# FFmpeg/FFmpeg

Hardware: AMD Instinct MI355X
Metric: swscale_nv12_1080p_to_4k_bicubic_Mpixels_per_s (higher is better)
Workload: dtype u8

## Files before the change

ffmpeg_amd/csrc/kernels/sws_up2.hip:

```cpp
#include <stdlib.h>
#include <type_traits>
#include <vector>

#include "common.h"
#include "sws_kernels.h"

typedef uint32_t up_u2 __attribute__((ext_vector_type(2)));
typedef uint32_t up_u3 __attribute__((ext_vector_type(3)));
typedef uint32_t up_u4 __attribute__((ext_vector_type(4)));
typedef uint32_t up_u8 __attribute__((ext_vector_type(8)));
typedef up_u3 __attribute__((aligned(4))) up_u3a;
typedef const uint8_t __attribute__((address_space(1))) *up_gcp;
typedef uint8_t __attribute__((address_space(1))) *up_gp;
typedef const up_u3a __attribute__((address_space(1))) *up_gc3;
typedef up_u2 __attribute__((address_space(1))) *up_g2;
typedef up_u4 __attribute__((aligned(4))) up_u4a;
typedef up_u2 __attribute__((aligned(4))) up_u2a;
typedef const up_u4a __attribute__((address_space(1))) *up_gc4;
typedef const up_u2a __attribute__((address_space(1))) *up_gc2;
typedef up_u4a __attribute__((address_space(1))) *up_g4;
typedef const up_u8 __attribute__((address_space(4))) *up_cc8;

struct UpRaw { uint32_t q[3]; };
struct UpRawH { uint32_t q[6]; };
// ... 217 lines not shown
#pragma unroll
    for (int i = 0; i < 8; i++)
        hprev[i] = 0;
    int kround = HB ? 1 << (vsh - 1) : 64 << 12;
    asm volatile("" : "+v"(kround));

    auto hpass = [&](const Raw &w, uint32_t (&Pnew)[8]) {
        int h[8];
        if (HB) {
            uint32_t v[6];
            constexpr int NQ = PAIR ? 6 : 4;
#pragma unroll
            for (int i = 0; i < NQ; i++)
                v[i] = w.q[i];
            if (border) {
                if (PAIR) {
                    const uint32_t q0 = w.q[0], q1 = w.q[1], q2 = w.q[2], q3 = w.q[3], q4 = w.q[4], q5 = w.q[5];
                    v[0] = lb ? q0 : rb ? q2 : q0; v[1] = lb ? q0 : rb ? q3 : q1; v[2] = lb ? q0 : rb ? q4 : q2;
                    v[3] = lb ? q1 : rb ? q5 : q3; v[4] = lb ? q2 : rb ? q5 : q4; v[5] = lb ? q3 : rb ? q5 : q5;
                } else {
                    const uint32_t q0 = w.q[0], q1 = w.q[1], q2 = w.q[2], q3 = w.q[3];
                    const uint32_t f0 = __builtin_amdgcn_perm(q0, q0, 0x01000100u), f3 = __builtin_amdgcn_perm(q3, q3, 0x03020302u);
                    v[0] = lb ? f0 : rb ? q1 : q0; v[1] = lb ? q0 : rb ? q2 : q1;
                    v[2] = lb ? q1 : rb ? q3 : q2; v[3] = lb ? q2 : rb ? f3 : q3;
                }
            }
            if (smsb) {
                typedef unsigned short up_h2 __attribute__((ext_vector_type(2)));
#pragma unroll
                for (int i = 0; i < NQ; i++)
                    v[i] = __builtin_bit_cast(uint32_t, __builtin_bit_cast(up_h2, v[i]) >> (unsigned short)smsb);
            }
            if (PAIR) {
                uint32_t a[5], b[5];
#pragma unroll
                for (int k = 0; k < 5; k++) {
                    a[k] = __builtin_amdgcn_perm(v[k + 1], v[k], 0x05040100u);
                    b[k] = __builtin_amdgcn_perm(v[k + 1], v[k], 0x07060302u);
                }
                int ha[4], hb[4];
                up_h4s(ha, a[0], a[1], a[1], a[2], a[2], a[3], a[3], a[4], cf, hsh);
                up_h4s(hb, b[0], b[1], b[1], b[2], b[2], b[3], b[3], b[4], cf, hsh);
#pragma unroll
                for (int i = 0; i < 4; i++) {
                    h[2 * i] = ha[i];
                    h[2 * i + 1] = hb[i];
                }
            } else {
                const uint32_t p0 = v[0], p2 = v[1], p4 = v[2], p6 = v[3];
                const uint32_t p1 = __builtin_amdgcn_alignbyte(v[1], v[0], 2), p3 = __builtin_amdgcn_alignbyte(v[2], v[1], 2);
                const uint32_t p5 = __builtin_amdgcn_alignbyte(v[3], v[2], 2);
                int hl[4], hh[4];
                up_h4s(hl, p0, p1, p1, p2, p2, p3, p3, p4, cf, hsh);
                up_h4s(hh, p2, p3, p3, p4, p4, p5, p5, p6, cf + 8, hsh);
#pragma unroll
                for (int i = 0; i < 4; i++) {
                    h[i] = hl[i];
                    h[4 + i] = hh[i];
                }
            }
#pragma unroll
            for (int i = 0; i < 8; i++) {
                Pnew[i] = __builtin_bit_cast(uint32_t, __builtin_amdgcn_cvt_pk_i16(hprev[i], h[i]));
                hprev[i] = h[i];
            }
            return;
        }
        uint32_t v0 = w.q[0], v1 = w.q[1], v2 = w.q[2];
        if (border) {
            const uint32_t f0 = __builtin_amdgcn_perm(w.q[0], w.q[0], fixl), f2 = __builtin_amdgcn_perm(w.q[2], w.q[2], fixr);
            v0 = lb ? f0 : rb ? w.q[1] : w.q[0];
            v1 = lb ? w.q[0] : rb ? w.q[2] : w.q[1];
            v2 = lb ? w.q[1] : rb ? f2 : w.q[2];
        }
        if (PAIR) {
            const uint32_t a0 = __builtin_amdgcn_perm(v1, v0, sA0), a1 = __builtin_amdgcn_perm(v1, v0, sA1);
            const uint32_t a2 = __builtin_amdgcn_perm(v1, v0, sA2), a3 = __builtin_amdgcn_perm(v2, v1, sA1);
            const uint32_t a4 = __builtin_amdgcn_perm(v2, v1, sA2);
            const uint32_t b0 = __builtin_amdgcn_perm(v1, v0, sB0), b1 = __builtin_amdgcn_perm(v1, v0, sB1);
            const uint32_t b2 = __builtin_amdgcn_perm(v1, v0, sB2), b3 = __builtin_amdgcn_perm(v2, v1, sB1);
            const uint32_t b4 = __builtin_amdgcn_perm(v2, v1, sB2);
            int ha[4], hb[4];
            if (SC) {
                up_h4c(ha, a0, a1, a1, a2, a2, a3, a3, a4, cE0, cE1, cO0, cO1);
                up_h4c(hb, b0, b1, b1, b2, b2, b3, b3, b4, cE0, cE1, cO0, cO1);
                if (border) {
                    const uint32_t *L = J.hco + 4, *R = J.hco + 10;
                    const int l0 = up_h1(a0, a2, L[0], L[1]), l1 = up_h1(a1, a3, L[2], L[3]), l2 = up_h1(a1, a3, L[4], L[5]);
                    const int m0 = up_h1(b0, b2, L[0], L[1]), m1 = up_h1(b1, b3, L[2], L[3]), m2 = up_h1(b1, b3, L[4], L[5]);
                    const int r1 = up_h1(a1, a3, R[0], R[1]), r2 = up_h1(a1, a3, R[2], R[3]), r3 = up_h1(a2, a4, R[4], R[5]);
                    const int q1 = up_h1(b1, b3, R[0], R[1]), q2 = up_h1(b1, b3, R[2], R[3]), q3 = up_h1(b2, b4, R[4], R[5]);
                    ha[0] = lb ? l0 : ha[0]; ha[1] = lb ? l1 : rb ? r1 : ha[1]; ha[2] = lb ? l2 : rb ? r2 : ha[2]; ha[3] = rb ? r3 : ha[3];
                    hb[0] = lb ? m0 : hb[0]; hb[1] = lb ? m1 : rb ? q1 : hb[1]; hb[2] = lb ? m2 : rb ? q2 : hb[2]; hb[3] = rb ? q3 : hb[3];
                }
            } else {
                up_h4(ha, a0, a1, a1, a2, a2, a3, a3, a4, cf);
                up_h4(hb, b0, b1, b1, b2, b2, b3, b3, b4, cf);
            }
#pragma unroll
            for (int i = 0; i < 4; i++) {
                h[2 * i] = ha[i];
                h[2 * i + 1] = hb[i];
            }
        } else {
            const uint32_t p0 = __builtin_amdgcn_perm(v1, v0, 0x0c030c02u), p1 = __builtin_amdgcn_perm(v1, v0, 0x0c040c03u);
            const uint32_t p2 = __builtin_amdgcn_perm(v1, v0, 0x0c050c04u), p3 = __builtin_amdgcn_perm(v1, v0, 0x0c060c05u);
            const uint32_t p4 = __builtin_amdgcn_perm(v1, v0, 0x0c070c06u), p5 = __builtin_amdgcn_perm(v2, v1, 0x0c040c03u);
            const uint32_t p6 = __builtin_amdgcn_perm(v2, v1, 0x0c050c04u);
            int hl[4], hh[4];
            if (SC) {
                up_h4c(hl, p0, p1, p1, p2, p2, p3, p3, p4, cE0, cE1, cO0, cO1);
                up_h4c(hh, p2, p3, p3, p4, p4, p5, p5, p6, cE0, cE1, cO0, cO1);
                if (border) {
                    const uint32_t *L = J.hco + 4, *R = J.hco + 10;
                    const int l0 = up_h1(p0, p2, L[0], L[1]), l1 = up_h1(p1, p3, L[2], L[3]), l2 = up_h1(p1, p3, L[4], L[5]);
                    const int r5 = up_h1(p3, p5, R[0], R[1]), r6 = up_h1(p3, p5, R[2], R[3]), r7 = up_h1(p4, p6, R[4], R[5]);
                    hl[0] = lb ? l0 : hl[0]; hl[1] = lb ? l1 : hl[1]; hl[2] = lb ? l2 : hl[2];
                    hh[1] = rb ? r5 : hh[1]; hh[2] = rb ? r6 : hh[2]; hh[3] = rb ? r7 : hh[3];
                }
            } else {
                up_h4(hl, p0, p1, p1, p2, p2, p3, p3, p4, cf);
                up_h4(hh, p2, p3, p3, p4, p4, p5, p5, p6, cf + 8);
            }
#pragma unroll
            for (int i = 0; i < 4; i++) {
                h[i] = hl[i];
                h[4 + i] = hh[i];
            }
        }
        if (RC) {
            const int rcc = J.rc_coeff, rco = J.rc_offset;
#pragma unroll
            for (int i = 0; i < 8; i++)
                h[i] = (__mul24(min(h[i], 32767), rcc) + rco) >> 14;
        }
#pragma unroll
        for (int i = 0; i < 8; i++) {
            Pnew[i] = __builtin_bit_cast(uint32_t, __builtin_amdgcn_cvt_pk_i16(hprev[i], h[i]));
            hprev[i] = h[i];
        }
    };

    Raw buf[D];
#pragma unroll
    for (int k = 0; k < D; k++)
        load_next(buf[k]);
#pragma unroll
    for (int k = 0; k < 3; k++) {
        hpass(buf[k % D], ring[k]);
        load_next(buf[k % D]);
    }

    const uint32_t *vt = J.vfv;
    for (int r = a; r < b; r += 6) {
        up_u8 c8[3];
#pragma unroll
        for (int q = 0; q < 3; q++)
            c8[q] = *(up_cc8)(vt + 4 * (r + 2 * q) - 4);
#pragma unroll
        for (int k = 0; k < 6; k++) {
            Raw &w = buf[(k + 3) % D];
            if constexpr (HB != 0) {
                const bool live = act && r + k < b;
                hpass(w, ring[k % 3]);
                const up_u8 cc = c8[k >> 1];
                const uint32_t fb01 = k & 1 ? cc.s4 : cc.s0, fb23 = k & 1 ? cc.s5 : cc.s1;
                const uint32_t fa01 = k & 1 ? cc.s6 : cc.s2, fa23 = k & 1 ? cc.s7 : cc.s3;
                const int y = 2 * (r + k) - 3;
                typedef unsigned short up_h2 __attribute__((ext_vector_type(2)));
                uint32_t o0[4], o1[4];
                up_v8h(o0, ring[(k + 1) % 3], ring[k % 3], fb01, fb23, kround, vsh, maxpk);
                uint32_t off = doff;
                asm volatile("" : "+v"(off));
#pragma unroll
                for (int i = 0; i < 4; i++)
                    o0[i] = __builtin_bit_cast(uint32_t, __builtin_bit_cast(up_h2, o0[i]) << (unsigned short)dmsb);
                if (live && y >= 0) {
                    up_u4 st; st.x = o0[0]; st.y = o0[1]; st.z = o0[2]; st.w = o0[3];
                    if (NTS) __builtin_nontemporal_store(st, (up_g4)((up_gp)dr + off));
                    else *(up_g4)((up_gp)dr + off) = st;
                }
                up_v8h(o1, ring[(k + 1) % 3], ring[k % 3], fa01, fa23, kround, vsh, maxpk);
#pragma unroll
                for (int i = 0; i < 4; i++)
                    o1[i] = __builtin_bit_cast(uint32_t, __builtin_bit_cast(up_h2, o1[i]) << (unsigned short)dmsb);
                if (live && y + 1 < dstH) {
                    up_u4 st; st.x = o1[0]; st.y = o1[1]; st.z = o1[2]; st.w = o1[3];
                    if (NTS) __builtin_nontemporal_store(st, (up_g4)((up_gp)(dr + dstride) + off));
                    else *(up_g4)((up_gp)(dr + dstride) + off) = st;
                }
                dr += 2 * dstride;
                asm("" : "+s"(dr));
                load_next(w);
                continue;
            }
            if (r + k < b) {
                if (!DBG_COPY)
                    hpass(w, ring[k % 3]);
                const up_u8 cc = c8[k >> 1];
                const uint32_t fb01 = k & 1 ? cc.s4 : cc.s0, fb23 = k & 1 ? cc.s5 : cc.s1;
                const uint32_t fa01 = k & 1 ? cc.s6 : cc.s2, fa23 = k & 1 ? cc.s7 : cc.s3;
                const int y = 2 * (r + k) - 3;
                uint32_t w0, w1, a0, a1;
                if (DBG_COPY) { w0 = w.q[0] + fb01; w1 = w.q[1] + fb23; a0 = w.q[1] + fa01; a1 = w.q[2] + fa23; }
                else up_v8(w0, w1, ring[(k + 1) % 3], ring[k % 3], fb01, fb23, kround);
                uint32_t off = doff;
                asm volatile("" : "+v"(off));
                if (act && y >= 0 && (!DBG_NOST || (w0 == 0x12345678u && w1 == 0x9abcdef0u))) {
                    up_u2 s; s.x = w0; s.y = w1;
                    if (NTS) __builtin_nontemporal_store(s, (up_g2)((up_gp)dr + off));
                    else *(up_g2)((up_gp)dr + off) = s;
                }
                if (!DBG_COPY)
                    up_v8(a0, a1, ring[(k + 1) % 3], ring[k % 3], fa01, fa23, kround);
                if (act && y + 1 < dstH && (!DBG_NOST || (a0 == 0x12345678u && a1 == 0x9abcdef0u))) {
                    up_u2 s; s.x = a0; s.y = a1;
                    if (NTS) __builtin_nontemporal_store(s, (up_g2)((up_gp)(dr + dstride) + off));
                    else *(up_g2)((up_gp)(dr + dstride) + off) = s;
                }
                dr += 2 * dstride;
                asm("" : "+s"(dr));
            }
            load_next(w);
        }
    }
}

template <int D, int VAR, int HB = 0, int RC = 0, int SC = 0>
__global__ __launch_bounds__(256) void k_sws_up2(FFHipUp2Args A)
{
    const int wave = __builtin_amdgcn_readfirstlane((int)(threadIdx.x >> 6));
    const int lane = threadIdx.x & 63;
    const uint32_t blk = sws_block_numbering(blockIdx.x, gridDim.x, A.xcd);
    const uint32_t gw = blk * 4u + (uint32_t)wave;
    if (gw >= (uint32_t)A.units_per_pack * (uint32_t)A.npacks)
        return;
    const int pack = (int)(gw / (uint32_t)A.units_per_pack);
    const int u = (int)(gw - (uint32_t)pack * (uint32_t)A.units_per_pack);
    int j = 0;
    if (A.njobs > 1 && u >= A.job[1].unit_begin) j = 1;
    if (A.njobs > 2 && u >= A.job[2].unit_begin) j = 2;
    const FFHipUp2Job &J = A.job[j];
    const int local = u - J.unit_begin;
    const int strip = local / J.upj, idx = local - strip * J.upj;
    const int nf = J.nfull << A.fshift;
    int frame0 = pack << A.fshift, fsh = 0, gbase;
    if (idx < nf) {
        const int fsub = idx / J.nfull;
        frame0 += fsub;
        gbase = (idx - fsub * J.nfull) * 64;
        if (frame0 >= A.nframes)
            return;
    } else {
        fsh = A.fshift;
        gbase = J.nfull * 64 + (idx - nf) * (64 >> fsh);
    }
    if (J.pair)
        up2_unit<1, D, VAR, HB, RC, SC>(J, frame0, fsh, gbase, strip, lane, A.nframes);
    else
        up2_unit<0, D, VAR, HB, RC, SC>(J, frame0, fsh, gbase, strip, lane, A.nframes);
}


int ffhip_up2_virtual_bank(const int16_t *filter, const int32_t *pos, int n_dst, int n_src, std::vector<uint32_t> *out)
{
    if (n_dst != 2 * n_src || n_src < 4)
        return 0;
    out->assign((size_t)n_dst * 2, 0);
    for (int x = 0; x < n_dst; x++) {
        const int s0 = (x >> 1) - 2 + (x & 1);
        int16_t v[4] = { 0, 0, 0, 0 };
        bool used[4] = { false, false, false, false };
        for (int i = 0; i < 4; i++) {
            const int16_t c = filter[(size_t)x * 4 + i];
            if (!c)
                continue;
            const int p = pos[x] + i;
            if (p < 0 || p >= n_src)
                return 0;
            int k = 0;
            for (; k < 4; k++) {
                int q = s0 + k;
                q = q < 0 ? 0 : q >= n_src ? n_src - 1 : q;
                if (q == p && !used[k])
                    break;
            }
            if (k == 4)
                return 0;
            used[k] = true;
            v[k] = c;
        }
        (*out)[2 * (size_t)x] = (uint16_t)v[0] | ((uint32_t)(uint16_t)v[1] << 16);
        (*out)[2 * (size_t)x + 1] = (uint16_t)v[2] | ((uint32_t)(uint16_t)v[3] << 16);
    }
    return 1;
}

int ffhip_up2_hco(const std::vector<uint32_t> &v, uint32_t out[16])
{
    const int n = (int)(v.size() / 2);
    if (n < 16 || (n & 1))
        return 0;
    for (int x = 3; x < n - 3; x++)
        if (v[2 * (size_t)x] != v[2 * (size_t)(4 + (x & 1))] || v[2 * (size_t)x + 1] != v[2 * (size_t)(4 + (x & 1)) + 1])
            return 0;
    for (int i = 0; i < 4; i++)
        out[i] = v[8 + i];
    for (int i = 0; i < 6; i++) {
        out[4 + i] = v[i];
        out[10 + i] = v[2 * (size_t)(n - 3) + i];
    }
    return 1;
}

void ffhip_up2_plan_job(FFHipUp2Job *j, int lanes_per_frame, int want)
{
    const int steps = j->srcH + 1;
    int n = cdiv(steps, want);
    int s = cdiv(cdiv(steps, n), 6) * 6;
    j->steps_per_strip = s;
    j->nstrips = cdiv(steps, s);
    if (lanes_per_frame == 64) {
        j->nfull = 0;
        j->upj = cdiv(j->ngroups, 64);
    } else {
        j->nfull = j->ngroups / 64;
        j->upj = j->nfull * (64 / lanes_per_frame) + cdiv(j->ngroups - j->nfull * 64, lanes_per_frame);
    }
}

int ffhip_launch_up2(FFHipUp2Args &A, int depth, int var, hipStream_t stream)
{
    if (A.nframes <= 0)
        return 0;
    int u = 0;
    for (int i = 0; i < A.njobs; i++) {
        A.job[i].unit_begin = u;
        u += A.job[i].upj * A.job[i].nstrips;
    }
    A.units_per_pack = u;
    A.npacks = (A.nframes + (1 << A.fshift) - 1) >> A.fshift;
    const long long waves = (long long)u * A.npacks;
    if (waves >= (1LL << 31)) {
        ffhip_set_error("ffhip_sws: batch too large for one launch (%lld waves)", waves);
        return FFHIP_EINVAL;
    }
    const dim3 grid((unsigned)((waves + 3) / 4)), block(256);
    if (A.job[0].hb_sdepth) {
        if (depth == 3 && !(var & 1))      hipLaunchKernelGGL((k_sws_up2<3, 0, 1>), grid, block, 0, stream, A);
        else if (depth == 3)               hipLaunchKernelGGL((k_sws_up2<3, 1, 1>), grid, block, 0, stream, A);
        else if (!(var & 1))               hipLaunchKernelGGL((k_sws_up2<6, 0, 1>), grid, block, 0, stream, A);
        else                               hipLaunchKernelGGL((k_sws_up2<6, 1, 1>), grid, block, 0, stream, A);
        LAUNCH_CHECK();
        return 0;
    }
    if (A.job[0].rc_coeff) {
        bool scr = var == 3;
        for (int i = 0; i < A.njobs; i++)
            scr = scr && A.job[i].hco_ok;
        if (scr && depth == 3)             hipLaunchKernelGGL((k_sws_up2<3, 1, 0, 1, 1>), grid, block, 0, stream, A);
        else if (scr)                      hipLaunchKernelGGL((k_sws_up2<6, 1, 0, 1, 1>), grid, block, 0, stream, A);
        else if (depth == 3)               hipLaunchKernelGGL((k_sws_up2<3, 0, 0, 1>), grid, block, 0, stream, A);
        else                               hipLaunchKernelGGL((k_sws_up2<6, 0, 0, 1>), grid, block, 0, stream, A);
        LAUNCH_CHECK();
        return 0;
    }
    bool sc = true;
    for (int i = 0; i < A.njobs; i++)
        sc = sc && A.job[i].hco_ok;
    if (var == 2 || var == 3) {
        if (!sc)
            var &= 1;
        else {
            if (var == 2 && depth == 3) hipLaunchKernelGGL((k_sws_up2<3, 0, 0, 0, 1>), grid, block, 0, stream, A);
            else if (var == 2)          hipLaunchKernelGGL((k_sws_up2<6, 0, 0, 0, 1>), grid, block, 0, stream, A);
            else if (depth == 3)        hipLaunchKernelGGL((k_sws_up2<3, 1, 0, 0, 1>), grid, block, 0, stream, A);
            else                        hipLaunchKernelGGL((k_sws_up2<6, 1, 0, 0, 1>), grid, block, 0, stream, A);
            LAUNCH_CHECK();
            return 0;
        }
    }
#define UP2_LAUNCH(DD, VV) hipLaunchKernelGGL((k_sws_up2<DD, VV>), grid, block, 0, stream, A)
#define UP2_CASE(VV) case VV: if (depth == 3) UP2_LAUNCH(3, VV); else UP2_LAUNCH(6, VV); break
    switch (var) {
    UP2_CASE(0);
    UP2_CASE(1);
    UP2_CASE(16); UP2_CASE(48); UP2_CASE(64);
    default:
        ffhip_set_error("ffhip_sws: exact-2x kernel variant %d is not built", var);
        return FFHIP_EINVAL;
    }
#undef UP2_CASE
#undef UP2_LAUNCH
    LAUNCH_CHECK();
    return 0;
}
```

ffmpeg_amd/csrc/sws_api.hip:

```cpp
#include <initializer_list>
#include <mutex>
#include <new>
#include <stdlib.h>
#include <string.h>
#include <utility>
#include <vector>

#include "kernels/common.h"
#include "kernels/sws_kernels.h"
#include "kernels/shim_arena.h"

struct DevBlock {
    void *p = nullptr;
    DevBlock() = default;
    DevBlock(const DevBlock &) = delete;
    DevBlock &operator=(const DevBlock &) = delete;
    DevBlock(DevBlock &&o) noexcept : p(o.p) { o.p = nullptr; }
    DevBlock &operator=(DevBlock &&o) noexcept { std::swap(p, o.p); return *this; }
    ~DevBlock() { if (p) (void)hipFree(p); }
};

static hipError_t grow(DevBlock &b, size_t &sz, size_t need)
{
    if (need <= sz)
// ... 1197 lines not shown
    uintptr_t al() const { return lal | cal; }
};

static SidePlanes side_planes(const void *const pl[4], const int stride[4], const size_t fp[4], int np, bool vfirst = false, int bytes = 1)
{
    SidePlanes s;
    for (int i = 0; i < np; i++) {
        (i ? s.cal : s.lal) |= (uintptr_t)pl[i] | (size_t)stride[i] | fp[i];
        s.neg = s.neg || stride[i] < 0;
        s.pos = s.pos && stride[i] > 0;
    }
    s.il = np == 2;
    for (int k = 0; k < (np > 1 ? 3 : 1); k++) {
        const int i = s.il && k ? 1 : k;
        s.p[k] = static_cast<uint8_t *>(const_cast<void *>(pl[i])) + (s.il && k && (k == 2) != vfirst ? bytes : 0);
        s.stride[k] = stride[i];
        s.fp[k] = fp[i];
    }
    s.pair = np > 1 ? static_cast<uint8_t *>(const_cast<void *>(pl[1])) : nullptr;
    s.swap = s.il && vfirst;
    return s;
}

struct PlaneJob {
    int which, plane;
    const uint8_t *src;
    uint8_t *dst;
    ptrdiff_t sstride, dstride;
    size_t sfp, dfp;
    int pair, swap, dswap;
};

template <class F> static void for_each_job(const SidePlanes &s, const SidePlanes &d, bool luma, bool chroma, F &&fill)
{
    if (luma)
        fill(PlaneJob{ 0, 0, s.p[0], d.p[0], s.stride[0], d.stride[0], s.fp[0], d.fp[0], 0, 0, 0 });
    if (!chroma)
        return;
    if (s.il)
        fill(PlaneJob{ 1, 1, s.pair, d.pair, s.stride[1], d.stride[1], s.fp[1], d.fp[1], 1, s.swap != d.swap, d.swap });
    else
        for (int k = 1; k < 3; k++)
            fill(PlaneJob{ 1, k, s.p[k], d.p[k], s.stride[k], d.stride[k], s.fp[k], d.fp[k], 0, 0, 0 });
}
template <class J> static void put_planes(J &j, const PlaneJob &q)
{
    j.src = q.src; j.dst = q.dst; j.sstride = q.sstride; j.dstride = q.dstride; j.sfp = q.sfp; j.dfp = q.dfp;
    j.pair = q.pair;
}

template <class A> static void put_src(A &a, const SidePlanes &s)
{
    for (int i = 0; i < 3; i++) {
        a.src[i] = i && s.il ? s.pair : s.p[i];
        a.sstride[i] = s.stride[i];
        a.sfp[i] = s.fp[i];
    }
}

static int up2_fshift(const FFHipUp2Args &U, int nframes)
{
    int best = -1;
    double bestw = 1e30;
    for (int fsft = 0; fsft <= 2; fsft++) {
        const int lpf = 64 >> fsft;
        bool fits = !(nframes < (1 << fsft) && fsft);
        double w = 0;
        for (int i = 0; i < U.njobs; i++) {
            const FFHipUp2Job &j = U.job[i];
            const unsigned long long span_s = (unsigned long long)((1 << fsft) - 1) * j.sfp + (unsigned long long)j.srcH * (size_t)(j.sstride < 0 ? -j.sstride : j.sstride);
            const unsigned long long span_d = (unsigned long long)((1 << fsft) - 1) * j.dfp + 2ull * j.srcH * (size_t)(j.dstride < 0 ? -j.dstride : j.dstride);
            if (span_s >= (1ull << 31) || span_d >= (1ull << 31))
                fits = false;
            const int nfull = fsft ? j.ngroups / 64 : 0;
            w += ((double)nfull + (double)cdiv(j.ngroups - nfull * 64, lpf) / (1 << fsft)) * j.srcH;
        }
        if (fits && w < bestw - 1e-9) {
            bestw = w;
            best = fsft;
        }
    }
    return best;
}

static int scale16(FFHipSwsContext *c, int nframes, const void *const src[4], const int srcStride[4], const size_t srcFramePitch[4],
                   void *const dst[4], const int dstStride[4], const size_t dstFramePitch[4], hipStream_t stream)
{
    const FFHipSwsTables &t = c->t;
    int sd = 8, sl = fmt_nv(t.srcFormat) ? 2 : 0, dd = 8, dl = fmt_nv(t.dstFormat) ? 2 : 0;
    (void)ffhip_pixfmt_hbd(t.srcFormat, &sd, &sl, nullptr, nullptr);
    (void)ffhip_pixfmt_hbd(t.dstFormat, &dd, &dl, nullptr, nullptr);
    const int ssz = sd > 8 ? 2 : 1, dsz = dd > 8 ? 2 : 1;
    const bool hrgb = fmt_rgb(t.dstFormat);
    for (int pl = 0; pl < (sl ? 2 : 3); pl++)
        if (!src[pl] || (srcStride[pl] % ssz) || (srcFramePitch[pl] % ssz) || ((uintptr_t)src[pl] % ssz))
            return FFHIP_EINVAL;
    for (int pl = 0; pl < (hrgb ? 1 : dl ? 2 : 3); pl++)
        if (!dst[pl] || (dstStride[pl] % dsz) || (dstFramePitch[pl] % dsz) || ((uintptr_t)dst[pl] % dsz))
            return FFHIP_EINVAL;
    const SidePlanes cs = side_planes(src, srcStride, srcFramePitch, sl ? 2 : 3, false, ssz);
    const SidePlanes d = side_planes(dst, dstStride, dstFramePitch, hrgb ? 1 : dl ? 2 : 3, false, dsz);
    SidePlanes ws = cs;
    ScratchLease wlease;
    bool widened = false;
    if (c->widen8 && (c->w16_ok || c->up2_ok || c->u32_ok) && d.pos && !(d.al() & 3) && cs.pos &&
        !knob_is(c->up2_ok ? "FFHIP_SWS_UP2" : "FFHIP_SWS_WALK16", '0')) {
        const int np = sl ? 2 : 3;
        const int wb[3] = { t.srcW, sl ? 2 * c->chrSrcW : c->chrSrcW, c->chrSrcW }, rows[3] = { t.srcH, c->chrSrcH, c->chrSrcH };
        size_t pitch[3], fp[3], off[3], need = 0;
        for (int pl = 0; pl < np; pl++) {
            pitch[pl] = ((size_t)2 * wb[pl] + 255) & ~(size_t)255;
            fp[pl] = pitch[pl] * (size_t)rows[pl];
            off[pl] = need;
            need += fp[pl] * (size_t)nframes;
        }
        HIP_TRY(acquire(c->widen_tmp, wlease, need, stream));
        const void *wsrc[4] = {};
        int wss[4] = {};
        size_t wsf[4] = {};
        for (int pl = 0; pl < np; pl++) {
            uint8_t *w = static_cast<uint8_t *>(c->widen_tmp.buf.p) + off[pl];
            const int r = ffhip_launch_sws_widen8(static_cast<const uint8_t *>(src[pl]), srcStride[pl], srcFramePitch[pl], w, (ptrdiff_t)pitch[pl], fp[pl],
                                                  wb[pl], rows[pl], nframes, stream);
            if (r < 0)
                return r;
            wsrc[pl] = w; wss[pl] = (int)pitch[pl]; wsf[pl] = fp[pl];
        }
        widened = true;
        sl = sl ? 1 : 0;
        ws = side_planes(wsrc, wss, wsf, np, false, 2);
    }
    const uintptr_t al = ws.al() | (hrgb ? 0 : d.al());
    const bool neg = ws.neg || d.neg;
    const int sw[2] = { t.srcW, c->chrSrcW }, sh[2] = { t.srcH, c->chrSrcH };
    if (c->up2_ok && (widened || !c->widen8) && !(al & 3) && !neg && !knob_is("FFHIP_SWS_UP2", '0')) {
        FFHipUp2Args U;
        memset(&U, 0, sizeof(U));
        U.nframes = nframes;
        U.xcd = 1;
        for_each_job(ws, d, true, true, [&](const PlaneJob &q) {
            FFHipUp2Job &j = U.job[U.njobs++];
            put_planes(j, q);
            j.swap = q.swap;
            j.srcW = sw[q.which]; j.srcH = sh[q.which];
            j.ngroups = q.pair ? j.srcW / 2 : j.srcW / 4;
            j.hfv = c->up2_h[q.which]; j.vfv = c->up2_v[q.which];
            j.hb_sdepth = sd; j.hb_ddepth = dd; j.hb_smsb = sl == 1 && !widened; j.hb_dmsb = dl == 1;
        });
        const int fs = up2_fshift(U, nframes);
        if (fs >= 0) {
            U.fshift = fs;
            for (int i = 0; i < U.njobs; i++)
                ffhip_up2_plan_job(&U.job[i], 64 >> U.fshift, 60);
            const char *ev2 = FFHIP_KNOB("FFHIP_UP2_VAR");
            return ffhip_launch_up2(U, knob_is("FFHIP_UP2_DEPTH", '3') ? 3 : 6, ev2 ? atoi(ev2) : 0, stream);
        }
    }
    if (c->dn2_ok && !(al & 3) && !neg && !knob_is("FFHIP_SWS_DOWN2", '0')) {
        FFHipDn2Args D;
        memset(&D, 0, sizeof(D));
        D.nframes = nframes;
        D.xcd = 1;
        for_each_job(cs, d, true, true, [&](const PlaneJob &q) {
            FFHipDn2Job &j = D.job[D.njobs++];
            put_planes(j, q);
            j.swap = q.swap;
            j.srcH = sh[q.which]; j.dstH = c->d[2 + q.which].n;
            j.ngroups = q.pair ? c->d[q.which].n / 2 : c->d[q.which].n / 4;
            j.hfv = c->dn2_h[q.which]; j.vfv = c->dn2_v[q.which];
            j.hb_sdepth = sd; j.hb_ddepth = dd; j.hb_smsb = sl == 1; j.hb_dmsb = dd > 8 && dl == 1;
            j.dither_off = q.plane == 2 ? 3 : 0;
            ffhip_down2_plan_job(&j, 32);
        });
        return ffhip_launch_down2(D, stream);
    }
    if (hrgb && !(c->w16_ok && !(al & 3) && !neg)) {
        ffhip_set_error("ffhip_sws: above 8 bits into packed RGB needs 4-byte aligned planes and pitches, top-down");
        return FFHIP_EINVAL;
    }
    if (c->d32_ok && !hrgb && !widened && !c->widen8 && !(al & 3) && !neg && !knob_is("FFHIP_SWS_DOWN32", '0')) {
        FFHipD32Args D;
        memset(&D, 0, sizeof(D));
        D.nframes = nframes;
        D.hb = 1; D.sdepth = sd; D.ddepth = dd; D.smsb = sl == 1; D.dmsb = dl == 1;
        D.ratio43 = c->d32_ok == 2;
        const int pin = D.ratio43 ? 4 : 3, pout = D.ratio43 ? 3 : 2;
        for_each_job(cs, d, true, true, [&](const PlaneJob &q) {
            FFHipD32Job &j = D.job[D.njobs++];
            put_planes(j, q);
            j.swap = q.swap;
            j.srcH = sh[q.which]; j.dstH = j.srcH / pin * pout;
            j.ngroups = q.pair ? c->d[q.which].n / pout : c->d[q.which].n / (2 * pout);
            j.hfv = c->d32_h[q.which]; j.vfv = c->d32_v[q.which];
            j.dither_off = q.plane == 2 ? 3 : 0;
        });
        return ffhip_launch_down32(D, stream);
    }
    if (c->u32_ok && !hrgb && (widened || !c->widen8) && !(al & 3) && !neg && !knob_is("FFHIP_SWS_UP32", '0')) {
        FFHipU32Args U;
        memset(&U, 0, sizeof(U));
        U.nframes = nframes;
        U.sdepth = sd; U.ddepth = dd; U.smsb = sl == 1 && !widened; U.dmsb = dl == 1;
        U.ratio43 = c->u32_ok == 2;
        const int pin = U.ratio43 ? 3 : 2, pout = U.ratio43 ? 4 : 3;
        for_each_job(ws, d, true, true, [&](const PlaneJob &q) {
            FFHipU32Job &j = U.job[U.njobs++];
            put_planes(j, q);
            j.srcH = sh[q.which]; j.dstH = j.srcH / pin * pout;
            j.ngroups = q.pair ? c->d[q.which].n / pout : c->d[q.which].n / (2 * pout);
            j.hfv = c->u32_h[q.which]; j.vfv = c->u32_v[q.which];
        });
        return ffhip_launch_up32(U, stream);
    }
    if (c->w16_ok && (widened || !c->widen8) && !(al & 3) && !neg && (hrgb || !knob_is("FFHIP_SWS_WALK16", '0'))) {
        SidePlanes wd = d;
        ScratchLease rlease;
        size_t ypitch = 0, cpitch = 0, yfp = 0, cfp = 0;
        if (hrgb) {
            ypitch = ((size_t)2 * t.dstW + 255) & ~(size_t)255; cpitch = ((size_t)(t.dstW / 2) + 255) & ~(size_t)255;
            yfp = ypitch * (size_t)t.dstH; cfp = cpitch * (size_t)t.dstH;
            HIP_TRY(acquire(c->rgb2_tmp, rlease, (yfp + 2 * cfp) * (size_t)nframes, stream));
            uint8_t *ty = static_cast<uint8_t *>(c->rgb2_tmp.buf.p);
            const void *x[4] = { ty, ty + yfp * (size_t)nframes, ty + (yfp + cfp) * (size_t)nframes, nullptr };
            const int xs[4] = { (int)ypitch, (int)cpitch, (int)cpitch, 0 };
            const size_t xf[4] = { yfp, cfp, cfp, 0 };
            wd = side_planes(x, xs, xf, 3);
        }
        FFHipW16Args W;
        memset(&W, 0, sizeof(W));
        W.nframes = nframes;
        W.ht = c->w16_ht; W.vt = c->w16_vt;
        W.sdepth = sd; W.ddepth = dd; W.smsb = sl == 1 && !widened; W.dmsb = dl == 1;
        W.flat_dither = hrgb ? (c->hrgb_seed0 ? 2 : 1) : c->flat_dither;
        int strip = 64;
        {
            const char *es = FFHIP_KNOB("FFHIP_W16_STRIP");
            auto waves = [&](int st) {
                const long long lum = (long long)cdiv(c->d[0].n, 256) * cdiv(c->d[2].n, st);
                const long long chr = (sl || dl) ? (long long)cdiv(c->d[1].n, 128) * cdiv(c->d[3].n, st)
                                                 : 2LL * cdiv(c->d[1].n, 256) * cdiv(c->d[3].n, st);
                return (lum + chr) * nframes;
            };
            if (es && atoi(es) > 0)
                strip = atoi(es) > 64 ? 64 : atoi(es);
            else
                while (strip > 16 && waves(strip) < 3 * 7168 / 2)
                    strip >>= 1;
        }
        auto job = [&](int which, int nch, int ch0) {
            FFHipW16Job &j = W.job[W.njobs++];
            j.nch = nch;
            j.sstep = which && ws.il ? 2 : 1; j.dstep = which && wd.il ? 2 : 1;
            j.dither_off = ch0 == 2 ? 3 : 0;
            for (int k = 0; k < nch; k++) {
                j.src[k] = ws.p[ch0 + k]; j.dst[k] = wd.p[ch0 + k];
                j.sstride[k] = ws.stride[ch0 + k]; j.dstride[k] = wd.stride[ch0 + k];
                j.sfp[k] = ws.fp[ch0 + k]; j.dfp[k] = wd.fp[ch0 + k];
            }
            j.srcH = sh[which];
            j.y16 = hrgb && !which;
            j.dstW = c->d[which].n; j.dstH = c->d[2 + which].n;
            j.hf = c->w16[which].filter; j.hp = c->w16[which].pos; j.vf = c->w16[2 + which].filter; j.vp = c->w16[2 + which].pos;
            j.srcW = sw[which];
            {
                const char *eg = FFHIP_KNOB("FFHIP_W16_STAGE");
                const int sp = c->w16_span[which][nch == 1 ? 0 : j.sstep == 2 ? 2 : 1];
                j.stage = sp > 0 && sp <= (eg && eg[0] == '1' ? 1024 : 512) && !(eg && eg[0] == '0');
            }
            ffhip_w16_plan_job(&j, strip);
        };
        if (!c->rgb_in_luma_done)
            job(0, 1, 0);
        if (ws.il || wd.il) {
            job(1, 2, 1);
        } else {
            job(1, 1, 1);
            job(1, 1, 2);
        }
        const int rw = ffhip_launch_walk16(W, stream);
        if (rw < 0 || !hrgb)
            return rw;
        FFHipY16RgbArgs Y;
        memset(&Y, 0, sizeof(Y));
        Y.y = wd.p[0]; Y.u = wd.p[1]; Y.v = wd.p[2];
        Y.dst = d.p[0];
        Y.ystride = (ptrdiff_t)ypitch; Y.cstride = (ptrdiff_t)cpitch; Y.dstride = d.stride[0];
        Y.yfp = yfp; Y.cfp = cfp; Y.dfp = d.fp[0];
        Y.w = t.dstW; Y.h = t.dstH; Y.nframes = nframes; Y.lay = rgb_layout(t.dstFormat); Y.k = c->k;
        return ffhip_launch_y16_rgb(Y, stream);
    }
    if (c->rgb_in_luma_done) {
        ffhip_set_error("ffhip_sws: internal: the converter pass wrote the luma plane but the walker does not run");
        return FFHIP_EINVAL;
    }
    FFHipScale16Args a;
    memset(&a, 0, sizeof(a));
    a.nplanes = 3;
    for (int pl = 0; pl < 3; pl++) {
        FFHipScale16Plane &p = a.pl[pl];
        const int sp = pl == 0 ? 0 : sl ? 1 : pl, dp = pl == 0 ? 0 : dl ? 1 : pl;
        p.src = static_cast<const uint8_t *>(src[sp]);
        p.dst = static_cast<uint8_t *>(dst[dp]);
        p.src_stride = srcStride[sp]; p.dst_stride = dstStride[dp];
        p.src_fp = srcFramePitch[sp]; p.dst_fp = dstFramePitch[dp];
        p.sdepth = sd; p.smsb = sl == 1; p.sstep = pl && sl ? 2 : 1; p.schan = pl && sl ? pl - 1 : 0;
        p.ddepth = dd; p.dmsb = dl == 1; p.dstep = pl && dl ? 2 : 1; p.dchan = pl && dl ? pl - 1 : 0;
        p.h = c->d[pl ? 1 : 0]; p.v = c->d[pl ? 3 : 2];
        p.dstW = p.h.n; p.dstH = p.v.n;
// ... 445 lines not shown
            Y.w = a.dstW; Y.h = a.dstH; Y.nframes = nframes; Y.lay = a.bgr; Y.k = c->k;
            return ffhip_launch_y16_rgb(Y, stream);
        }
        return ffhip_launch_scale_rgb(a, stream);
    }

    FFHipScalePlaneArgs l = c->lum, ch = c->chr;
    l.src[0] = l.src[1] = s.p[0]; l.src_stride[0] = l.src_stride[1] = s.stride[0];
    l.src_fp[0] = l.src_fp[1] = s.fp[0]; l.src_step = 1;
    l.dst[0] = l.dst[1] = d.p[0]; l.dst_stride[0] = l.dst_stride[1] = d.stride[0];
    l.dst_fp[0] = l.dst_fp[1] = d.fp[0]; l.dst_step = 1;
    l.nframes = nframes;
    for (int k = 0; k < 2; k++) {
        ch.src[k] = s.p[1 + k]; ch.src_stride[k] = s.stride[1 + k]; ch.src_fp[k] = s.fp[1 + k];
        ch.dst[k] = d.p[1 + k]; ch.dst_stride[k] = d.stride[1 + k]; ch.dst_fp[k] = d.fp[1 + k];
    }
    ch.src_step = s.il ? 2 : 1;
    ch.dst_step = d.il ? 2 : 1;
    ch.nframes = nframes;

    if (c->c420_ok && !fast_off && topdown) {
        FFHipCopy420Args K;
        memset(&K, 0, sizeof(K));
        K.nframes = nframes;
        const int cw = c->d[1].n, chh = c->d[3].n;
        {
            FFHipCopy420Job &j = K.job[K.njobs++];
            j.src[0] = s.p[0]; j.sstride[0] = s.stride[0]; j.sfp[0] = s.fp[0];
            j.dst = d.p[0]; j.dstride = d.stride[0]; j.dfp = d.fp[0];
            j.kind = 0; j.wbytes = t.dstW; j.rows = t.dstH;
        }
        if (d.il) {
            FFHipCopy420Job &j = K.job[K.njobs++];
            j.dst = d.pair; j.dstride = d.stride[1]; j.dfp = d.fp[1];
            j.wbytes = 2 * cw; j.rows = chh;
            if (s.il) {
                j.src[0] = s.pair; j.sstride[0] = s.stride[1]; j.sfp[0] = s.fp[1];
                j.kind = d.swap == s.swap ? 0 : 3;
            } else {
                j.kind = 2;
                for (int k = 0; k < 2; k++) {
                    const int sp = d.swap ? 2 - k : 1 + k;
                    j.src[k] = s.p[sp]; j.sstride[k] = s.stride[sp]; j.sfp[k] = s.fp[sp];
                }
            }
        } else {
            for (int k = 0; k < 2; k++) {
                FFHipCopy420Job &j = K.job[K.njobs++];
                j.dst = d.p[1 + k]; j.dstride = d.stride[1 + k]; j.dfp = d.fp[1 + k];
                j.wbytes = cw; j.rows = chh;
                if (s.il) {
                    j.src[0] = s.pair; j.sstride[0] = s.stride[1]; j.sfp[0] = s.fp[1];
                    j.kind = 1; j.k = s.swap ? !k : k;
                } else {
                    j.src[0] = s.p[1 + k]; j.sstride[0] = s.stride[1 + k]; j.sfp[0] = s.fp[1 + k];
                    j.kind = 0;
                }
            }
        }
        return ffhip_launch_copy420(K, stream);
    }
    if (c->mix_dn2 && !fast_off && topdown && !((s.cal | d.cal) & 3)) {
        FFHipCopy420Args K;
        memset(&K, 0, sizeof(K));
        K.nframes = nframes;
        FFHipCopy420Job &kj = K.job[K.njobs++];
        kj.src[0] = s.p[0]; kj.sstride[0] = s.stride[0]; kj.sfp[0] = s.fp[0];
        kj.dst = d.p[0]; kj.dstride = d.stride[0]; kj.dfp = d.fp[0];
        kj.kind = 0; kj.wbytes = t.dstW; kj.rows = t.dstH;
        const int r1 = ffhip_launch_copy420(K, stream);
        if (r1 < 0)
            return r1;
        FFHipDn2Args D;
        memset(&D, 0, sizeof(D));
        D.nframes = nframes;
        D.xcd = 1;
        for_each_job(s, d, false, true, [&](const PlaneJob &q) {
            FFHipDn2Job &j = D.job[D.njobs++];
            put_planes(j, q);
            j.srcH = c->chrSrcH; j.dstH = c->d[3].n; j.ngroups = c->d[1].n / 4;
            j.hfv = c->dn2_h[1]; j.vfv = c->dn2_v[1];
            ffhip_down2_plan_job(&j, 32);
        });
        return ffhip_launch_down2(D, stream);
    }
    if (!(al & 3) && c->u32_ok && !neg && !c->luma_pass && !knob_is("FFHIP_SWS_UP32", '0') ) {
        FFHipU32Args U;
        memset(&U, 0, sizeof(U));
        U.nframes = nframes;
        U.bytes = 1;
        U.ratio43 = c->u32_ok == 2;
        const int no = U.ratio43 ? 16 : 12;
        for_each_job(s, d, true, true, [&](const PlaneJob &q) {
            const FFHipScalePlaneArgs &p = q.which ? ch : l;
            FFHipU32Job &j = U.job[U.njobs++];
            put_planes(j, q);
            j.srcH = p.srcH; j.dstH = p.dstH;
            j.ngroups = q.pair ? p.dstW / (no / 2) : p.dstW / no;
            j.hfv = c->u32_h[q.which]; j.vfv = c->u32_v[q.which];
        });
        return ffhip_launch_up32(U, stream);
    }
    if (c->cw_ok && !fast_off) {
        if (!(al & 3) && (c->up2_ok || (c->mix_up2 && !c->luma_pass && topdown)) && !knob_is("FFHIP_SWS_UP2", '0') && !knob_is("FFHIP_SWS_MFMA", '1')) {
            FFHipUp2Args U;
            memset(&U, 0, sizeof(U));
            U.nframes = nframes;
            if (c->mix_up2) {
                FFHipCopy420Args K;
                memset(&K, 0, sizeof(K));
                K.nframes = nframes;
                FFHipCopy420Job &kj = K.job[K.njobs++];
                kj.src[0] = s.p[0]; kj.sstride[0] = s.stride[0]; kj.sfp[0] = s.fp[0];
                kj.dst = d.p[0]; kj.dstride = d.stride[0]; kj.dfp = d.fp[0];
                kj.kind = 0; kj.wbytes = l.dstW; kj.rows = l.dstH;
                const int r1 = ffhip_launch_copy420(K, stream);
                if (r1 < 0)
                    return r1;
            }
            for_each_job(s, d, !c->mix_up2, !c->luma_pass, [&](const PlaneJob &q) {
                const FFHipScalePlaneArgs &p = q.which ? ch : l;
                FFHipUp2Job &j = U.job[U.njobs++];
                put_planes(j, q);
                j.swap = q.swap;
                j.srcW = p.srcW; j.srcH = p.srcH;
                j.ngroups = q.pair ? p.srcW / 2 : p.srcW / 4;
                j.hfv = c->up2_h[q.which]; j.vfv = c->up2_v[q.which];
                j.rc_coeff = p.rc_coeff; j.rc_offset = p.rc_offset;
                j.hco_ok = c->up2_hco_ok[q.which];
                memcpy(j.hco, c->up2_hco[q.which], sizeof(j.hco));
            });
            const char *ef = FFHIP_KNOB("FFHIP_UP2_FSHIFT"), *es = FFHIP_KNOB("FFHIP_UP2_STRIP"), *ed = FFHIP_KNOB("FFHIP_UP2_DEPTH");
            const char *ev2 = FFHIP_KNOB("FFHIP_UP2_VAR"), *ex = FFHIP_KNOB("FFHIP_UP2_XCD");
            U.xcd = ex ? atoi(ex) : 1;
            const int fs = up2_fshift(U, nframes);
            U.fshift = ef && ef[0] >= '0' && ef[0] <= '2' ? ef[0] - '0' : fs < 0 ? 0 : fs;
            bool jneg = false;
            for (int i = 0; i < U.njobs; i++)
                jneg = jneg || U.job[i].sstride < 0 || U.job[i].dstride < 0;
            if (!jneg) {
                static const int wants[] = { 60, 36, 24, 12 };
                for (int w = 0; w < 4; w++) {
                    long long u = 0;
                    for (int i = 0; i < U.njobs; i++) {
                        ffhip_up2_plan_job(&U.job[i], 64 >> U.fshift, es && atoi(es) > 0 ? atoi(es) : wants[w]);
                        u += (long long)U.job[i].upj * U.job[i].nstrips;
                    }
                    if ((es && atoi(es) > 0) || u * ((nframes + (1 << U.fshift) - 1) >> U.fshift) >= 8192)
                        break;
                }
                bool scal = true;
                for (int i = 0; i < U.njobs; i++)
                    scal = scal && U.job[i].hco_ok;
                return ffhip_launch_up2(U, ed ? (ed[0] == '6' ? 6 : 3) : scal && !U.job[0].rc_coeff ? 6 : 3, ev2 ? atoi(ev2) : scal ? 3 : 0, stream);
            }
        }
        if (!(al & 3) && !c->up2_rc) {
            if (c->mf_ok && knob_is("FFHIP_SWS_MFMA", '1')) {
                const char *est = FFHIP_KNOB("FFHIP_MF_STRIP");
                FFHipMfArgs M;
                memset(&M, 0, sizeof(M));
                M.nframes = nframes;
                for_each_job(s, d, true, !c->luma_pass, [&](const PlaneJob &q) {
                    const FFHipScalePlaneArgs &p = q.which ? ch : l;
                    FFHipMfJob &j = M.job[M.njobs++];
                    put_planes(j, q);
                    j.dst_swap = q.dswap;
                    j.srcH = p.srcH; j.dstW = p.dstW; j.dstH = p.dstH;
                    j.tiles = c->mf_tiles[q.which]; j.vf = c->dn[2 + q.which].filter; j.vp = c->dn[2 + q.which].pos; j.ys = c->mf_ys[q.which];
                    j.ntiles = c->mf_ntiles[q.which];
                    j.ncb = cdiv(j.ntiles, 16);
                    const int want = est && atoi(est) > 0 ? atoi(est) : 540;
                    const int ns = cdiv(p.dstH, want);
                    j.strip_rows = cdiv(p.dstH, ns);
                    j.nstrips = cdiv(p.dstH, j.strip_rows);
                });
                return ffhip_launch_mfma(M, stream);
            }
            const char *eg = FFHIP_KNOB("FFHIP_CW_LUMA_GROUPS"), *ep = FFHIP_KNOB("FFHIP_CW_PLAIN");
            const char *ed = FFHIP_KNOB("FFHIP_CW_DEPTH"), *es = FFHIP_KNOB("FFHIP_CW_STRIP");
            const int lg = (eg && eg[0] == '1') || (ep && ep[0] == '1') ? 1 : 2;
            const int depth = ed && ed[0] == '3' ? 3 : 6;
            static const int strips[] = { 120, 60, 40, 24 };
            int gpl[3], strip = 120;
            FFHipCwArgs A;
            memset(&A, 0, sizeof(A));
            A.nframes = nframes;
            A.flags = ep && ep[0] == '1' ? 1 : 0;
            if (c->cw_opt && !A.flags && !knob_is("FFHIP_CW_OPT", '0'))
                A.flags |= 2;
            if ((A.flags & 2) && c->cw_dup && !knob_is("FFHIP_CW_DUP", '0'))
                A.flags |= 4;
            auto bank = [&](FFHipCwJob &j, const FFHipScalePlaneArgs &p) {
                const int which = &p == &ch ? 1 : 0;
                j.srcW = p.srcW; j.srcH = p.srcH; j.dstW = p.dstW; j.dstH = p.dstH;
                j.hf = c->dn[which].filter; j.hp = c->dn[which].pos; j.vf = c->dn[2 + which].filter; j.vp = c->dn[2 + which].pos;
            };
            FFHipCwJob &jl = A.job[0];
            bank(jl, l);
            jl.kind = lg == 2 ? 1 : 0;
            jl.src[0] = s.p[0]; jl.sstride[0] = s.stride[0]; jl.sfp[0] = s.fp[0];
            jl.dst[0] = d.p[0]; jl.dstride[0] = d.stride[0]; jl.dfp[0] = d.fp[0];
            gpl[0] = lg;
            A.njobs = 1;
            if (c->luma_pass) {
            } else if (!s.il && !d.il) {
                for (int k = 1; k < 3; k++) {
                    FFHipCwJob &j = A.job[A.njobs++];
                    bank(j, ch);
                    j.kind = jl.kind;
                    j.src[0] = s.p[k]; j.sstride[0] = s.stride[k]; j.sfp[0] = s.fp[k];
                    j.dst[0] = d.p[k]; j.dstride[0] = d.stride[k]; j.dfp[0] = d.fp[k];
                    gpl[A.njobs - 1] = lg;
                }
            } else {
                FFHipCwJob &j = A.job[A.njobs++];
                bank(j, ch);
                j.kind = s.il && d.il ? 2 : s.il ? 3 : 4;
                for (int k = 0; k < 2; k++) {
                    j.src[k] = s.il && !k ? s.pair : s.p[1 + k]; j.sstride[k] = s.stride[1 + k]; j.sfp[k] = s.fp[1 + k];
                    j.dst[k] = d.il && !k ? d.pair : d.p[1 + k]; j.dstride[k] = d.stride[1 + k]; j.dfp[k] = d.fp[1 + k];
                }
                j.src_swap = s.swap;
                j.dst_swap = d.swap;
                gpl[A.njobs - 1] = 1;
            }
            for (int i = 0; i < 4; i++) {
                strip = es && atoi(es) > 0 ? atoi(es) : strips[i];
                long long u = 0;
                for (int k = 0; k < A.njobs; k++) {
                    ffhip_cw_plan_job(&A.job[k], gpl[k], strip);
                    u += (long long)A.job[k].ncb * A.job[k].nstrips;
                }
                if ((es && atoi(es) > 0) || u * nframes >= 4096)
                    break;
            }
            return ffhip_launch_colwalk(A, lg, depth, stream);
        }
    }
    if (!(al & 3) && c->dn2_ok && !neg && !knob_is("FFHIP_SWS_DOWN2", '0') && !fast_off) {
        FFHipDn2Args D;
        memset(&D, 0, sizeof(D));
        D.nframes = nframes;
        const char *es = FFHIP_KNOB("FFHIP_DN2_STRIP");
        D.xcd = !knob_is("FFHIP_DN2_XCD", '0');
        for_each_job(s, d, true, !c->luma_pass, [&](const PlaneJob &q) {
            const FFHipScalePlaneArgs &p = q.which ? ch : l;
            FFHipDn2Job &j = D.job[D.njobs++];
            put_planes(j, q);
            j.swap = q.swap;
            j.srcH = p.srcH; j.dstH = p.dstH;
            j.ngroups = q.pair ? p.dstW / 2 : p.dstW / 4;
            j.hfv = c->dn2_h[q.which]; j.vfv = c->dn2_v[q.which];
            ffhip_down2_plan_job(&j, es && atoi(es) > 0 ? atoi(es) : 32);
        });
        return ffhip_launch_down2(D, stream);
    }
    if (!(al & 3) && c->d32_ok && !neg && !c->luma_pass && !knob_is("FFHIP_SWS_DOWN32", '0')  && !fast_off) {
        FFHipD32Args D;
        memset(&D, 0, sizeof(D));
        D.nframes = nframes;
        for_each_job(s, d, true, true, [&](const PlaneJob &q) {
            const FFHipScalePlaneArgs &p = q.which ? ch : l;
            FFHipD32Job &j = D.job[D.njobs++];
            put_planes(j, q);
            j.swap = q.swap;
            j.srcH = p.srcH; j.dstH = p.dstH;
            j.ngroups = q.pair ? p.dstW / 4 : p.dstW / 8;
            j.hfv = c->d32_h[q.which]; j.vfv = c->d32_v[q.which];
        });
        return ffhip_launch_down32(D, stream);
    }
    const char *ew = FFHIP_KNOB("FFHIP_SWS_WIDE");
    if (c->lw_ok && !(ew && ew[0] == '0') && !(fast_off && !(ew && ew[0] == '1')) && !(al & 3)) {
        FFHipLwArgs W;
        memset(&W, 0, sizeof(W));
        W.nframes = nframes; W.ht = c->lw_ht; W.vt = c->lw_vt;
        auto wbank = [&](FFHipLwJob &j, const FFHipScalePlaneArgs &p, int which) {
            j.srcW = p.srcW; j.srcH = p.srcH; j.dstW = p.dstW; j.dstH = p.dstH;
            j.hf = c->dw[which].filter; j.hp = c->dw[which].pos; j.vf = c->dw[2 + which].filter; j.vp = c->dw[2 + which].pos;
            ffhip_lw_plan_job(&j);
        };
        if (c->luma_pass) {
        } else if (!s.il && !d.il) {
            for (int k = 1; k < 3; k++) {
                FFHipLwJob &j = W.job[W.njobs++];
                j.src[0] = s.p[k]; j.sstride[0] = s.stride[k]; j.sfp[0] = s.fp[k];
                j.dst[0] = d.p[k]; j.dstride[0] = d.stride[k]; j.dfp[0] = d.fp[k];
                wbank(j, ch, 1);
            }
        } else {
            FFHipLwJob &j = W.job[W.njobs++];
            j.pair = 1; j.sil = s.il; j.dil = d.il;
            for (int k = 0; k < 2; k++) {
                j.src[k] = s.il && !k ? s.pair : s.p[1 + k]; j.sstride[k] = s.stride[1 + k]; j.sfp[k] = s.fp[1 + k];
                j.dst[k] = d.il && !k ? d.pair : d.p[1 + k]; j.dstride[k] = d.stride[1 + k]; j.dfp[k] = d.fp[1 + k];
            }
            j.src_swap = s.swap;
            j.dst_swap = d.swap;
            wbank(j, ch, 1);
        }
        FFHipLwJob &jl = W.job[W.njobs++];
        jl.src[0] = s.p[0]; jl.sstride[0] = s.stride[0]; jl.sfp[0] = s.fp[0];
        jl.dst[0] = d.p[0]; jl.dstride[0] = d.stride[0]; jl.dfp[0] = d.fp[0];
        wbank(jl, l, 0);
        return ffhip_launch_lwalk(W, stream);
    }
// ... 359 lines not shown
```

Before: 2.820 million.

## Add bounds-check-free fast trip for interior rows of exact 2x upscale

Wraps the per-six-row body in a lambda templated on a FAST flag. When the whole wave is active, interior rows run a variant with the liveness and edge store predicates compiled out, and only the head and tail rows go through the checked path. It also uniformises the strip and frame indices with readfirstlane so they stay in scalar registers. The launch code gains an 'exact' variant bit that is now on by default, and the default pipeline depth changes (6 when chroma pairs are present, otherwise 3). This adds more template instantiations and a split loop in exchange for removing per-row branching and predication.

```diff
diff --git a/ffmpeg_amd/csrc/kernels/sws_up2.hip b/ffmpeg_amd/csrc/kernels/sws_up2.hip
--- a/ffmpeg_amd/csrc/kernels/sws_up2.hip
+++ b/ffmpeg_amd/csrc/kernels/sws_up2.hip
@@ -393,7 +393,8 @@
     }
 
     const uint32_t *vt = J.vfv;
-    for (int r = a; r < b; r += 6) {
+    auto trip = [&](auto fast, const int r) {
+        constexpr bool FAST = decltype(fast)::value;
         up_u8 c8[3];
 #pragma unroll
         for (int q = 0; q < 3; q++)
@@ -402,7 +403,7 @@
         for (int k = 0; k < 6; k++) {
             Raw &w = buf[(k + 3) % D];
             if constexpr (HB != 0) {
-                const bool live = act && r + k < b;
+                const bool live = FAST || (act && r + k < b);
                 hpass(w, ring[k % 3]);
                 const up_u8 cc = c8[k >> 1];
                 const uint32_t fb01 = k & 1 ? cc.s4 : cc.s0, fb23 = k & 1 ? cc.s5 : cc.s1;
@@ -416,7 +417,7 @@
 #pragma unroll
                 for (int i = 0; i < 4; i++)
                     o0[i] = __builtin_bit_cast(uint32_t, __builtin_bit_cast(up_h2, o0[i]) << (unsigned short)dmsb);
-                if (live && y >= 0) {
+                if (FAST || (live && y >= 0)) {
                     up_u4 st; st.x = o0[0]; st.y = o0[1]; st.z = o0[2]; st.w = o0[3];
                     if (NTS) __builtin_nontemporal_store(st, (up_g4)((up_gp)dr + off));
                     else *(up_g4)((up_gp)dr + off) = st;
@@ -425,7 +426,7 @@
 #pragma unroll
                 for (int i = 0; i < 4; i++)
                     o1[i] = __builtin_bit_cast(uint32_t, __builtin_bit_cast(up_h2, o1[i]) << (unsigned short)dmsb);
-                if (live && y + 1 < dstH) {
+                if (FAST || (live && y + 1 < dstH)) {
                     up_u4 st; st.x = o1[0]; st.y = o1[1]; st.z = o1[2]; st.w = o1[3];
                     if (NTS) __builtin_nontemporal_store(st, (up_g4)((up_gp)(dr + dstride) + off));
                     else *(up_g4)((up_gp)(dr + dstride) + off) = st;
@@ -435,7 +436,7 @@
                 load_next(w);
                 continue;
             }
-            if (r + k < b) {
+            if (FAST || r + k < b) {
                 if (!DBG_COPY)
                     hpass(w, ring[k % 3]);
                 const up_u8 cc = c8[k >> 1];
@@ -447,14 +448,14 @@
                 else up_v8(w0, w1, ring[(k + 1) % 3], ring[k % 3], fb01, fb23, kround);
                 uint32_t off = doff;
                 asm volatile("" : "+v"(off));
-                if (act && y >= 0 && (!DBG_NOST || (w0 == 0x12345678u && w1 == 0x9abcdef0u))) {
+                if (FAST || (act && y >= 0 && (!DBG_NOST || (w0 == 0x12345678u && w1 == 0x9abcdef0u)))) {
                     up_u2 s; s.x = w0; s.y = w1;
                     if (NTS) __builtin_nontemporal_store(s, (up_g2)((up_gp)dr + off));
                     else *(up_g2)((up_gp)dr + off) = s;
                 }
                 if (!DBG_COPY)
                     up_v8(a0, a1, ring[(k + 1) % 3], ring[k % 3], fa01, fa23, kround);
-                if (act && y + 1 < dstH && (!DBG_NOST || (a0 == 0x12345678u && a1 == 0x9abcdef0u))) {
+                if (FAST || (act && y + 1 < dstH && (!DBG_NOST || (a0 == 0x12345678u && a1 == 0x9abcdef0u)))) {
                     up_u2 s; s.x = a0; s.y = a1;
                     if (NTS) __builtin_nontemporal_store(s, (up_g2)((up_gp)(dr + dstride) + off));
                     else *(up_g2)((up_gp)(dr + dstride) + off) = s;
@@ -463,6 +464,30 @@
                 asm("" : "+s"(dr));
             }
             load_next(w);
+        }
+    };
+
+    constexpr bool EXACT = (VAR & 4) && !(VAR & (16 | 32 | 64));
+    if constexpr (!EXACT) {
+        for (int r = a; r < b; r += 6)
+            trip(std::false_type(), r);
+    } else {
+        const bool full = __builtin_amdgcn_ballot_w64(act) == ~0ull;
+        const int f1 = full ? min(b, srcH + 1) : 0;
+        int r = a;
+#pragma nounroll
+        for (int pass = 0; pass < 2; pass++) {
+            const int e = pass ? b : min(b, a == 1 ? a + 6 : a);
+#pragma nounroll
+            for (; r < e; r += 6)
+                trip(std::false_type(), r);
+            if (!pass && r + 5 < f1) {
+                trip(std::true_type(), r);
+                r += 6;
+#pragma nounroll
+                for (; r + 5 < f1; r += 6)
+                    trip(std::true_type(), r);
+            }
         }
     }
 }
@@ -476,18 +501,18 @@
     const uint32_t gw = blk * 4u + (uint32_t)wave;
     if (gw >= (uint32_t)A.units_per_pack * (uint32_t)A.npacks)
         return;
-    const int pack = (int)(gw / (uint32_t)A.units_per_pack);
+    const int pack = __builtin_amdgcn_readfirstlane((int)(gw / (uint32_t)A.units_per_pack));
     const int u = (int)(gw - (uint32_t)pack * (uint32_t)A.units_per_pack);
     int j = 0;
     if (A.njobs > 1 && u >= A.job[1].unit_begin) j = 1;
     if (A.njobs > 2 && u >= A.job[2].unit_begin) j = 2;
     const FFHipUp2Job &J = A.job[j];
     const int local = u - J.unit_begin;
-    const int strip = local / J.upj, idx = local - strip * J.upj;
+    const int strip = __builtin_amdgcn_readfirstlane(local / J.upj), idx = local - strip * J.upj;
     const int nf = J.nfull << A.fshift;
     int frame0 = pack << A.fshift, fsh = 0, gbase;
     if (idx < nf) {
-        const int fsub = idx / J.nfull;
+        const int fsub = __builtin_amdgcn_readfirstlane(idx / J.nfull);
         frame0 += fsub;
         gbase = (idx - fsub * J.nfull) * 64;
         if (frame0 >= A.nframes)
@@ -587,11 +612,18 @@
         return FFHIP_EINVAL;
     }
     const dim3 grid((unsigned)((waves + 3) / 4)), block(256);
+    const bool exact = var >= 0 && var < 8 && (var & 4);
+    if (exact)
+        var &= ~4;
+#define UP2_K(DD, VV, ...) hipLaunchKernelGGL((k_sws_up2<DD, VV, ##__VA_ARGS__>), grid, block, 0, stream, A)
+#define UP2_PICK(VV, ...)                                                                                    \
+    do {                                                                                                     \
+        if (depth == 3) { if (exact) UP2_K(3, (VV) | 4, ##__VA_ARGS__); else UP2_K(3, VV, ##__VA_ARGS__); } \
+        else            { if (exact) UP2_K(6, (VV) | 4, ##__VA_ARGS__); else UP2_K(6, VV, ##__VA_ARGS__); } \
+    } while (0)
     if (A.job[0].hb_sdepth) {
-        if (depth == 3 && !(var & 1))      hipLaunchKernelGGL((k_sws_up2<3, 0, 1>), grid, block, 0, stream, A);
-        else if (depth == 3)               hipLaunchKernelGGL((k_sws_up2<3, 1, 1>), grid, block, 0, stream, A);
-        else if (!(var & 1))               hipLaunchKernelGGL((k_sws_up2<6, 0, 1>), grid, block, 0, stream, A);
-        else                               hipLaunchKernelGGL((k_sws_up2<6, 1, 1>), grid, block, 0, stream, A);
+        if (var & 1) UP2_PICK(1, 1);
+        else         UP2_PICK(0, 1);
         LAUNCH_CHECK();
         return 0;
     }
@@ -599,10 +631,8 @@
         bool scr = var == 3;
         for (int i = 0; i < A.njobs; i++)
             scr = scr && A.job[i].hco_ok;
-        if (scr && depth == 3)             hipLaunchKernelGGL((k_sws_up2<3, 1, 0, 1, 1>), grid, block, 0, stream, A);
-        else if (scr)                      hipLaunchKernelGGL((k_sws_up2<6, 1, 0, 1, 1>), grid, block, 0, stream, A);
-        else if (depth == 3)               hipLaunchKernelGGL((k_sws_up2<3, 0, 0, 1>), grid, block, 0, stream, A);
-        else                               hipLaunchKernelGGL((k_sws_up2<6, 0, 0, 1>), grid, block, 0, stream, A);
+        if (scr) UP2_PICK(1, 0, 1, 1);
+        else     UP2_PICK(0, 0, 1);
         LAUNCH_CHECK();
         return 0;
     }
@@ -613,26 +643,24 @@
         if (!sc)
             var &= 1;
         else {
-            if (var == 2 && depth == 3) hipLaunchKernelGGL((k_sws_up2<3, 0, 0, 0, 1>), grid, block, 0, stream, A);
-            else if (var == 2)          hipLaunchKernelGGL((k_sws_up2<6, 0, 0, 0, 1>), grid, block, 0, stream, A);
-            else if (depth == 3)        hipLaunchKernelGGL((k_sws_up2<3, 1, 0, 0, 1>), grid, block, 0, stream, A);
-            else                        hipLaunchKernelGGL((k_sws_up2<6, 1, 0, 0, 1>), grid, block, 0, stream, A);
+            if (var == 2) UP2_PICK(0, 0, 0, 1);
+            else          UP2_PICK(1, 0, 0, 1);
             LAUNCH_CHECK();
             return 0;
         }
     }
-#define UP2_LAUNCH(DD, VV) hipLaunchKernelGGL((k_sws_up2<DD, VV>), grid, block, 0, stream, A)
-#define UP2_CASE(VV) case VV: if (depth == 3) UP2_LAUNCH(3, VV); else UP2_LAUNCH(6, VV); break
-    switch (var) {
-    UP2_CASE(0);
-    UP2_CASE(1);
+#define UP2_CASE(VV) case VV: if (depth == 3) UP2_K(3, VV); else UP2_K(6, VV); break
+    switch (exact ? -1 - var : var) {
+    case 0: case -1: UP2_PICK(0); break;
+    case 1: case -2: UP2_PICK(1); break;
     UP2_CASE(16); UP2_CASE(48); UP2_CASE(64);
     default:
         ffhip_set_error("ffhip_sws: exact-2x kernel variant %d is not built", var);
         return FFHIP_EINVAL;
     }
 #undef UP2_CASE
-#undef UP2_LAUNCH
+#undef UP2_PICK
+#undef UP2_K
     LAUNCH_CHECK();
     return 0;
 }
diff --git a/ffmpeg_amd/csrc/sws_api.hip b/ffmpeg_amd/csrc/sws_api.hip
--- a/ffmpeg_amd/csrc/sws_api.hip
+++ b/ffmpeg_amd/csrc/sws_api.hip
@@ -1373,8 +1373,11 @@
             U.fshift = fs;
             for (int i = 0; i < U.njobs; i++)
                 ffhip_up2_plan_job(&U.job[i], 64 >> U.fshift, 60);
-            const char *ev2 = FFHIP_KNOB("FFHIP_UP2_VAR");
-            return ffhip_launch_up2(U, knob_is("FFHIP_UP2_DEPTH", '3') ? 3 : 6, ev2 ? atoi(ev2) : 0, stream);
+            const char *ev2 = FFHIP_KNOB("FFHIP_UP2_VAR"), *ed = FFHIP_KNOB("FFHIP_UP2_DEPTH");
+            bool pairs = false;
+            for (int i = 0; i < U.njobs; i++)
+                pairs = pairs || U.job[i].pair;
+            return ffhip_launch_up2(U, ed ? (ed[0] == '3' ? 3 : 6) : pairs ? 6 : 3, ev2 ? atoi(ev2) : 4, stream);
         }
     }
     if (c->dn2_ok && !(al & 3) && !neg && !knob_is("FFHIP_SWS_DOWN2", '0')) {
@@ -2126,7 +2129,7 @@
                 bool scal = true;
                 for (int i = 0; i < U.njobs; i++)
                     scal = scal && U.job[i].hco_ok;
-                return ffhip_launch_up2(U, ed ? (ed[0] == '6' ? 6 : 3) : scal && !U.job[0].rc_coeff ? 6 : 3, ev2 ? atoi(ev2) : scal ? 3 : 0, stream);
+                return ffhip_launch_up2(U, ed ? (ed[0] == '6' ? 6 : 3) : 3, ev2 ? atoi(ev2) : scal ? 7 : 4, stream);
             }
         }
         if (!(al & 3) && !c->up2_rc) {
```

Result: no change. 2.844 million, median of 6 (+0.8%).
